# i3drobotics/i3dr_stereo_camera-ros

Measured on AMD Instinct MI355X. Metric: stereo pairs/sec + ms/frame, 1920×1080 D=256 8-path SGM, 1/2/4/8 MI355X, higher is better.
Workload: dtype u8

## Files before the change

### i3dr_stereo_camera-ros_amd/csrc/census_sgm.hip

```cpp
#include "sgm_device.h"

#include <atomic>
#include <string>

#ifndef SGM_WPE
#define SGM_WPE 4
#endif
#ifndef SGM_WPE32
#define SGM_WPE32 4
#endif
#ifndef SGM_NT_STORE
#define SGM_NT_STORE 1
#endif
#ifndef SGM_NT_LOAD
#define SGM_NT_LOAD 1
#endif
#ifndef SGM_EXP
#define SGM_EXP 0
#endif
#if SGM_EXP != 0 && !defined(SGM_EXPERIMENT_BUILD)
#error "SGM_EXP builds give invalid results: define SGM_EXPERIMENT_BUILD as well (never in a release build)"
#endif
#ifndef SGM_LRPRIO_HW
#define SGM_LRPRIO_HW 37
// ... 124 lines not shown
    } else if constexpr (DPL == 4) {
        const uint32_t v = __builtin_amdgcn_perm(L[1], L[0], 0x06040200u);
        if constexpr (SGM_NT_STORE) __builtin_nontemporal_store(v, (uint32_t*)dst);
        else *(uint32_t*)dst = v;
    } else if constexpr (DPL == 8) {
        typedef unsigned int v2u __attribute__((ext_vector_type(2)));
        const v2u v = {__builtin_amdgcn_perm(L[1], L[0], 0x06040200u), __builtin_amdgcn_perm(L[3], L[2], 0x06040200u)};
        if constexpr (SGM_NT_STORE) __builtin_nontemporal_store(v, (v2u*)dst);
        else *(v2u*)dst = v;
    } else {
        typedef unsigned int v4u __attribute__((ext_vector_type(4)));
#pragma unroll
        for (int q = 0; q < DPL / 16; q++) {
            const v4u v = {__builtin_amdgcn_perm(L[8 * q + 1], L[8 * q + 0], 0x06040200u),
                           __builtin_amdgcn_perm(L[8 * q + 3], L[8 * q + 2], 0x06040200u),
                           __builtin_amdgcn_perm(L[8 * q + 5], L[8 * q + 4], 0x06040200u),
                           __builtin_amdgcn_perm(L[8 * q + 7], L[8 * q + 6], 0x06040200u)};
            v4u* d = (v4u*)(q == 0 ? dst : dst_hi);
            if constexpr (SGM_NT_STORE) __builtin_nontemporal_store(v, d);
            else *d = v;
        }
    }
}

constexpr uint32_t kBaseP = 0x6400u, kBaseP2 = 0x64006400u;
constexpr uint32_t kInfP = 0x7000u, kInfP2 = 0x70007000u;

__device__ __forceinline__ uint32_t pk_min3_p(uint32_t a, uint32_t b, uint32_t c)
{
    typedef _Float16 h2_t __attribute__((ext_vector_type(2)));
    const h2_t r = __builtin_elementwise_minimum(
        __builtin_elementwise_minimum(__builtin_bit_cast(h2_t, a), __builtin_bit_cast(h2_t, b)), __builtin_bit_cast(h2_t, c));
    return __builtin_bit_cast(uint32_t, r);
}
__device__ __forceinline__ uint32_t pk_max(uint32_t a, uint32_t b) { return as_u(__builtin_elementwise_max(as_v2(a), as_v2(b))); }

__device__ __forceinline__ uint32_t bcnt_acc(uint32_t x, uint32_t acc)
{
    uint32_t r;
    asm("v_bcnt_u32_b32 %0, %1, %2" : "=v"(r) : "v"(x), "v"(acc));
    return r;
}
__device__ __forceinline__ uint32_t ham_acc(uint64_t a, uint64_t b, uint32_t acc)
{
    const uint64_t x = a ^ b;
    return bcnt_acc((uint32_t)(x >> 32), bcnt_acc((uint32_t)x, acc));
}

__device__ __forceinline__ uint32_t pk_shl(uint32_t a, int sh)
{
    return as_u(as_v2(a) << (u16x2_t){(unsigned short)sh, (unsigned short)sh});
}
__device__ __forceinline__ uint32_t pk_subs(uint32_t a, uint32_t b) { return as_u(__builtin_elementwise_sub_sat(as_v2(a), as_v2(b))); }
template <int DPL, int LPL = 16>
__device__ __forceinline__ void p16_relative(const uint32_t (&Labs)[DPL / 2], uint32_t (&Lr)[DPL / 2])
{
    constexpr int M = DPL / 2;
    uint32_t mn = Labs[0];
#pragma unroll
    for (int i = 1; i < M; i += 2) mn = (i + 1 < M) ? pk_min3_p(mn, Labs[i], Labs[i + 1]) : pk_min(mn, Labs[i]);
    mn = line_min_u32<LPL>(pk_min(mn, alignbit16(mn, mn)));
    uint32_t off = mn - kBaseP2;
    asm("" : "+v"(off));
#pragma unroll
    for (int i = 0; i < M; i++) Lr[i] = Labs[i] - off;
}

template <int DPL, bool EXACT, int LPL = 16, typename F>
__device__ __forceinline__ void p16_step(uint32_t (&Lr)[DPL / 2], uint64_t cl, F crk, uint32_t P1P1, uint32_t P2P2,
                                         const uint32_t (&imask)[DPL / 2], uint32_t (&Labs)[DPL / 2])
{
    constexpr int M = DPL / 2;
    constexpr int SH = LPL == 8 ? 2 : 1;
    uint32_t q[M];
#pragma unroll
    for (int i = 0; i < M; i++) q[i] = Lr[i] + P1P1;
    const uint32_t X = LPL == 32 ? line32_shr1(q[M - 1], kInfP2) : row_shr_n<SH>(q[M - 1], kInfP2);
    const uint32_t Y = LPL == 32 ? line32_shl1(q[0], kInfP2) : row_shl_n<SH>(q[0], kInfP2);
    uint32_t Oprev = alignbit16(q[0], X);
#pragma unroll
    for (int i = 0; i < M; i++) {
        const uint32_t Onext = (i + 1 < M) ? alignbit16(q[i + 1], q[i]) : alignbit16(Y, q[M - 1]);
        const uint32_t t = pk_min(pk_min3_p(Oprev, Onext, Lr[i]), P2P2);
        const uint32_t c1 = ham_acc(cl, crk(2 * i + 1), 0u);
        uint32_t L = ham_acc(cl, crk(2 * i), t) + (c1 << 16);
        if (!EXACT) L = pk_max(L, imask[i]);
        Labs[i] = L;
        Oprev = Onext;
    }
    p16_relative<DPL, LPL>(Labs, Lr);
}

template <int DPL, bool EXACT>
__device__ __forceinline__ void make_imask(int p, int D, uint32_t (&imask)[DPL / 2], uint32_t (&start)[DPL / 2])
{
#pragma unroll
    for (int i = 0; i < DPL / 2; i++) {
        const int d = p * DPL + 2 * i;
        imask[i] = EXACT ? 0u : ((d < D ? 0u : kInfP) | (d + 1 < D ? 0u : kInfP << 16));
        start[i] = imask[i] | kBaseP2;
    }
}

struct PathLaunch16 {
    int xb_lo[6];
    const uint8_t* bnd[2];
    size_t bnd_slot;
};
__host__ __device__ constexpr int bnd_slot_of(int dir) { return dir <= 1 ? 0 : (dir == 2 || dir == 4 ? 1 : 2); }
__host__ __device__ constexpr uint32_t path_item(int dir, int lb, int f = 0)
{
    return ((uint32_t)dir << 24) | ((uint32_t)f << 22) | (uint32_t)lb;
}

template <typename T>
__device__ __forceinline__ T pick4(const T (&a)[kMaxGroup], int f)
{
    return f == 0 ? a[0] : f == 1 ? a[1] : f == 2 ? a[2] : a[3];
}

constexpr int kWG = 256;

template <int DPL16>
struct LineCfg {
    static constexpr int LPL = (DPL16 == 32 && SGM_P32) ? 32 : 16;
    static constexpr int DPL = DPL16 * 16 / LPL;
    static constexpr int HROWS = 4 * (64 / LPL);
};

struct HChunk16 {
    uint64_t cl, inj;
};

template <int DPL, int DX, int LPL>
__device__ __forceinline__ HChunk16 hload16(const uint64_t* cLr, const uint64_t* cRr, const Geom& g, int chunk,
                                            int i16)
{
    const int i = chunk * 16 + i16;
    const int x = DX > 0 ? g.minX1 + i : g.maxX1 - 1 - i;
    HChunk16 c;
    c.cl = cLr[min(max(x, 0), g.W - 1)];
    const int xr = DX > 0 ? x + 1 - g.minD : x - g.minD - LPL * DPL;
    c.inj = cRr[min(max(xr, 0), g.W - 1)];
    return c;
}

template <int DPL, bool EXACT, int DX, bool PRIO = false, int LPL = 16>
__device__ __forceinline__ void p16_horiz(const uint64_t* __restrict__ cL, const uint64_t* __restrict__ cR,
                                          uint8_t* __restrict__ V, uint8_t* __restrict__ trash, const Geom& g,
                                          int y0)
{
    static_assert(LPL == 16 || LPL == 32, "horizontal scans: 16- or 32-lane lines");
    constexpr int M = DPL / 2;
    constexpr int U = DPL > 16 ? DPL : 16;
    const int lane = threadIdx.x & 63;
    const int r = lane / LPL, p = lane % LPL;
    const int y = y0 + r;
    const bool rowok = y < g.H;
    const int yc = min(y, g.H - 1);
    const uint64_t* cLr = cL + (size_t)yc * g.W;
    const uint64_t* cRr = cR + (size_t)yc * g.W;
    uint32_t imask[M], start[M];
    make_imask<DPL, EXACT>(p, g.D, imask, start);
    const uint32_t P1P1 = (uint32_t)g.P1 * 0x10001u, P2P2 = ((uint32_t)g.P2 + kBaseP) * 0x10001u;
    const int n = g.width1;
    const int xfirst = DX > 0 ? g.minX1 : g.maxX1 - 1;
    uint64_t cr[DPL];
#pragma unroll
    for (int k = 0; k < DPL; k++) cr[k] = cRr[min(max(xfirst - g.minD - p * DPL - k, 0), g.W - 1)];
    uint32_t Lr[M];
#pragma unroll
    for (int i = 0; i < M; i++) Lr[i] = start[i];
    uint8_t* rowbase = V + (size_t)yc * g.width1 * g.D + p * DPL;
    uint8_t* tr = trash + lane * DPL;
    const bool lane_ok = rowok && (EXACT || p * DPL < g.D);
    const bool hi_ok = EXACT || p * DPL + 16 < g.D;
    HChunk16 cur = hload16<DPL, DX, LPL>(cLr, cRr, g, 0, lane & 15);
    HChunk16 nxt = cur;
    for (int b = 0; b * U < n; b++) {
        if constexpr (PRIO) lr_prio(((n - b * U) * SGM_LRPRIO_HW) >> 6, g.H);
        static_for<0, U>([&](auto tc) {
            constexpr int t = decltype(tc)::value;
            if constexpr (t % 16 == 0) nxt = hload16<DPL, DX, LPL>(cLr, cRr, g, (b * U + t) / 16 + 1, lane & 15);
            const int i = b * U + t;
            const uint64_t cl = row_bcast_u64<t % 16>(cur.cl);
            const uint64_t inj = row_bcast_u64<t % 16>(cur.inj);
            uint32_t Labs[M];
            p16_step<DPL, EXACT, LPL>(Lr, cl, [&](int k) { return cr[DX > 0 ? ((k - t) % DPL + DPL) % DPL : (k + t) % DPL]; },
                                      P1P1, P2P2, imask, Labs);
            const int x1 = DX > 0 ? i : n - 1 - i;
            const bool ok = lane_ok && i < n;
            uint8_t* dst = ok ? rowbase + (size_t)x1 * g.D : tr;
            store_pairs<DPL>(dst, (ok && hi_ok) ? dst + 16 : tr + 16, Labs);
            if constexpr (DX > 0) {
                constexpr int ph = ((DPL - 1 - t) % DPL + DPL) % DPL;
                cr[ph] = LPL == 32 ? line32_shr1_u64(cr[ph], inj) : row_shr1_u64(cr[ph], inj);
            } else {
                constexpr int ph = t % DPL;
                cr[ph] = LPL == 32 ? line32_shl1_u64(cr[ph], inj) : row_shl1_u64(cr[ph], inj);
            }
            if constexpr (t % 16 == 15) cur = nxt;
        });
    }
}

template <int DPL, int LPL>
struct RowSeg {
    static constexpr int NL = kWG / LPL;
    static constexpr int NSEG = LPL * DPL + NL - 1;
    static constexpr int NPAD = LPL >= 16 ? NSEG + NSEG / 16 + 1 : NSEG + 4 * (NSEG / 32) + 4;
    static constexpr int NTOT = NSEG + NL;
    static constexpr int NLOAD = (NTOT + kWG - 1) / kWG;
    static constexpr int BUF = NPAD + NL + kWG;
    static __device__ __forceinline__ int phys(int e) { return LPL >= 16 ? e + (e >> 4) : e + 4 * (e >> 5); }
};
template <int DPL16>
// ... 53 lines not shown
    }
}

template <int DPL, bool EXACT, int LPL>
__device__ __forceinline__ void p16_seed(const uint8_t* src, const uint32_t (&imask)[DPL / 2], uint32_t (&Lr)[DPL / 2])
{
    uint32_t wd[(DPL + 3) / 4], Labs[DPL / 2];
    wload<DPL>(src, wd);
#pragma unroll
    for (int i = 0; i < DPL / 2; i++) {
        const uint32_t pr = __builtin_amdgcn_perm(0u, wd[i / 2], (i & 1) ? 0x0c030c02u : 0x0c010c00u);
        Labs[i] = pr | kBaseP2;
        if (!EXACT) Labs[i] = pk_max(Labs[i], imask[i]);
    }
    p16_relative<DPL, LPL>(Labs, Lr);
}

struct UpWta {
    const uint8_t* vols;
    size_t vol_bytes;
    uint64_t* res;
};
struct WtaPix { int best, minS, d16; bool rej; };
template <int DPL, bool EXACT>
__device__ __forceinline__ WtaPix wta_pix16(const uint32_t (&E)[(DPL + 3) / 4], const uint32_t (&O)[(DPL + 3) / 4],
                                            int p, const Geom& g, float inv_u, uint32_t* srow);
template <int DPL, bool EXACT>
__device__ __forceinline__ void wta_emask(int p, const Geom& g, uint32_t (&emaskE)[(DPL + 3) / 4],
                                          uint32_t (&emaskO)[(DPL + 3) / 4]);
template <int DPL>
__host__ __device__ constexpr size_t upwta_lds_bytes() { return (size_t)8 * 2 * RowSeg<DPL, 16>::BUF + (size_t)16 * 32 * ((DPL + 3) / 4) * 4; }

template <int DPL, bool EXACT, int LPL, bool FUSE = false, bool PRIO = false>
__device__ __forceinline__ void p16_rows(const uint64_t* __restrict__ cL, const uint64_t* __restrict__ cR,
                                         uint8_t* __restrict__ V, uint8_t* __restrict__ trash, const Geom& g, int dir,
                                         int xb, const PathLaunch16& pl, uint64_t* lds, const UpWta& uw = UpWta{})
{
    static_assert(!FUSE || LPL == 16, "up+WTA blocks use 16 lanes per line (the WTA layout)");
    using RS = RowSeg<DPL, LPL>;
    constexpr int M = DPL / 2;
    constexpr int NL = RS::NL;
    const int tid = threadIdx.x;
    const int lane = tid & 63, w = tid >> 6;
    const int r = lane >> 4;
    const int p = LPL == 32 ? lane & 31 : LPL == 16 ? lane & 15 : (lane & 15) >> 1;
    const int j = LPL == 32 ? 2 * w + (lane >> 5) : LPL == 16 ? 4 * w + r : 8 * w + 2 * r + (lane & 1);
    const int rx = dir_rx(dir), ry = dir_ry(dir);
    int s0, s1;
    if (rx == 0) { s0 = 0; s1 = g.H; }
    else if (rx > 0) { s0 = max(0, g.minX1 - xb - (NL - 1)); s1 = min(g.H, g.maxX1 - xb); }
    else { s0 = max(0, xb - g.maxX1 + 1); s1 = min(g.H, xb + NL - g.minX1); }
    if (s0 >= s1) return;
    uint32_t imask[M], start[M];
    make_imask<DPL, EXACT>(p, g.D, imask, start);
    const uint32_t P1P1 = (uint32_t)g.P1 * 0x10001u, P2P2 = ((uint32_t)g.P2 + kBaseP) * 0x10001u;
    uint32_t Lr[M];
#pragma unroll
    for (int i = 0; i < M; i++) Lr[i] = start[i];
    bool pv = false;
    const uint8_t* bnd = pl.bnd[ry > 0 ? 0 : 1];
    if (bnd && s0 == 0) {
        const int x = xb + j, xp = x - rx;
        const bool cont = x >= g.minX1 && x < g.maxX1 && xp >= g.minX1 && xp < g.maxX1;
        const int xs = min(max(xp, g.minX1), g.maxX1 - 1) - g.minX1;
        uint32_t Ls[M];
        p16_seed<DPL, EXACT, LPL>(bnd + bnd_slot_of(dir) * pl.bnd_slot + (size_t)xs * g.D + p * DPL, imask, Ls);
#pragma unroll
        for (int i = 0; i < M; i++) Lr[i] = cont ? Ls[i] : Lr[i];
        pv = cont;
    }
    const bool lane_act = EXACT || p * DPL < g.D;
    const bool hi_ok = EXACT || p * DPL + 16 < g.D;
    uint8_t* const tr = trash + (tid & 63) * DPL;
    const int e_hi = j + (LPL - p) * DPL - 1;

    uint64_t* buf0 = lds;
    uint64_t* buf1 = lds + RS::BUF;
    uint64_t R0[RS::NLOAD], R1[RS::NLOAD], R2[RS::NLOAD], R3[RS::NLOAD];
    const SegAddr<DPL, LPL> sa = seg_addr<DPL, LPL>(cL, cR, g, tid);
    seg_load<DPL, LPL>(R0, sa, g, rx, ry, xb, s0);
    seg_store<DPL, LPL>(buf0, R0, tid);
    seg_load<DPL, LPL>(R1, sa, g, rx, ry, xb, min(s0 + 1, s1 - 1));
    seg_load<DPL, LPL>(R2, sa, g, rx, ry, xb, min(s0 + 2, s1 - 1));
    seg_load<DPL, LPL>(R3, sa, g, rx, ry, xb, min(s0 + 3, s1 - 1));
    __syncthreads();

    constexpr int NWD = (DPL + 3) / 4;
    uint32_t vw[7][NWD], emaskE[NWD], emaskO[NWD];
    uint32_t* srow = (uint32_t*)(lds + 2 * RS::BUF) + j * 32 * NWD;
    const float inv_u = 1.0f / (float)max(100 - g.uniq, 1);
    const uint32_t voff = (uint32_t)((min(max(xb + j, g.minX1), g.maxX1 - 1) - g.minX1) * g.D + (lane_act ? p * DPL : 0));
    auto vload = [&](int s) {
        const uint8_t* rb = uw.vols + (size_t)max(g.H - 1 - s, 0) * g.width1 * g.D;
#pragma unroll
        for (int k = 0; k < 7; k++) wload_buf<DPL>(rb + (size_t)(k == 0 ? 0 : k + 1) * uw.vol_bytes, voff, vw[k]);
    };
    if constexpr (FUSE) {
        wta_emask<DPL, EXACT>(p, g, emaskE, emaskO);
        vload(s0);
    }
    auto step = [&](int s, const uint64_t* bufc) {
        const int x = xb + j + rx * s;
        const bool valid = s < s1 && x >= g.minX1 && x < g.maxX1;
        const int y = ry > 0 ? s : g.H - 1 - s;
        const uint64_t cl = bufc[RS::NPAD + j];
        uint32_t Labs[M];
        uint32_t E[NWD], O[NWD];
        if constexpr (FUSE) {
#pragma unroll
            for (int jj = 0; jj < NWD; jj++) {
                uint32_t e = 0, o = 0;
#pragma unroll
                for (int k = 0; k < 7; k++) {
                    e += vw[k][jj] & 0x00FF00FFu;
                    o += __builtin_amdgcn_perm(0u, vw[k][jj], 0x0c030c01u);
                }
                asm("" : "+v"(e), "+v"(o));
                E[jj] = e;
                O[jj] = o;
            }
        }
        const uint32_t P2x = pv ? P2P2 : kBaseP2;
        if constexpr (FUSE) __builtin_amdgcn_sched_barrier(0);
        p16_step<DPL, EXACT, LPL>(Lr, cl, [&](int k) { return bufc[RS::phys(e_hi - k)]; }, P1P1, P2x, imask, Labs);
        if constexpr (FUSE) {
            __builtin_amdgcn_sched_barrier(0);
#pragma unroll
            for (int jj = 0; jj < NWD; jj++) {
                const uint32_t a = Labs[2 * jj], b = 2 * jj + 1 < M ? Labs[2 * jj + 1] : 0u;
                E[jj] = (E[jj] + __builtin_amdgcn_perm(b, a, 0x0c040c00u)) | emaskE[jj];
                O[jj] = (O[jj] + __builtin_amdgcn_perm(b, a, 0x0c060c02u)) | emaskO[jj];
            }
            vload(s + 1);
            __builtin_amdgcn_sched_barrier(0);
            const WtaPix px = wta_pix16<DPL, EXACT>(E, O, p, g, inv_u, srow);
            const uint64_t v = (uint64_t)(uint16_t)(px.rej ? g.invalid : px.d16) |
                               ((uint64_t)(uint16_t)(px.rej ? -1 : px.best) << 16) | ((uint64_t)(uint16_t)px.minS << 32);
            const __amdgpu_buffer_rsrc_t rr =
                __builtin_amdgcn_make_buffer_rsrc((void*)(uw.res + (size_t)y * g.W), 0, g.W * 8, 0x00020000);
            typedef unsigned int v2u __attribute__((ext_vector_type(2)));
            __builtin_amdgcn_raw_buffer_store_b64(__builtin_bit_cast(v2u, v), rr,
                                                  (valid && p == 0) ? (uint32_t)x * 8u : 0x80000000u, 0, 2);
        } else {
            const bool ok = valid && lane_act && !((SGM_EXP & 2) && dir == 1);
            uint8_t* const vrow = V + (size_t)min(max(y, 0), g.H - 1) * g.width1 * g.D;
            uint8_t* const dst = ok ? vrow + (uint32_t)((x - g.minX1) * g.D + p * DPL) : tr;
            store_pairs<DPL>(dst, (ok && hi_ok) ? dst + 16 : tr + 16, Labs);
        }
        pv = valid;
    };
    auto body = [&](int s, const uint64_t* bcur, uint64_t* bnext, uint64_t (&Rnext)[RS::NLOAD],
                    uint64_t (&Rfree)[RS::NLOAD]) {
        seg_load<DPL, LPL>(Rfree, sa, g, rx, ry, xb, min(s + 4, s1 - 1));
        step(s, bcur);
        seg_store<DPL, LPL>(bnext, Rnext, tid);
        __syncthreads();
    };
    for (int s = s0; s < s1; s += 4) {
        if constexpr (PRIO) lr_prio(rx != 0 ? ((s1 - s) * SGM_LRPRIO_DIAG) >> 6 : s1 - s, g.H);
        body(s, buf0, buf1, R1, R0);
        body(s + 1, buf1, buf0, R2, R1);
        body(s + 2, buf0, buf1, R3, R2);
        body(s + 3, buf1, buf0, R0, R3);
    }
}

template <int DPL>
__host__ __device__ constexpr int rows_lds_codes() { return 2 * RowSeg<RowsCfg<DPL>::DPL, RowsCfg<DPL>::LPL>::BUF; }

template <int DPL, bool EXACT, bool PRIO = false>
__device__ __forceinline__ void paths_block16(const PathFrames& pf, size_t vol_bytes, size_t trash_off,
                                              const Geom& g, const PathLaunch16& pl, uint32_t it, uint64_t* lds)
{
    using RC = RowsCfg<DPL>;
    using HC = LineCfg<DPL>;
    const int dir = (int)(it >> 24);
    const int f = (int)((it >> 22) & 3u);
    const int lb = (int)(it & 0x3FFFFFu);
    if (f >= pf.n || ((pf.skip_dirs >> dir) & 1u)) return;
    const uint64_t* cL = pick4(pf.cL, f);
    const uint64_t* cR = pick4(pf.cR, f);
    uint8_t* V = pick4(pf.vols, f) + (size_t)dir * vol_bytes;
    uint8_t* trash = V + trash_off;
    const int y0 = lb * HC::HROWS + (64 / HC::LPL) * (threadIdx.x >> 6);
    if (dir == 6) p16_horiz<HC::DPL, EXACT, 1, PRIO, HC::LPL>(cL, cR, V, trash, g, y0);
    else if (dir == 7) p16_horiz<HC::DPL, EXACT, -1, PRIO, HC::LPL>(cL, cR, V, trash, g, y0);
    else p16_rows<RC::DPL, EXACT, RC::LPL, false, PRIO>(cL, cR, V, trash, g, dir, pl.xb_lo[dir] + lb * RC::NL, pl, lds);
}

__device__ __forceinline__ void trace_record(uint64_t* trace, uint64_t tag, uint64_t t0)
{
    const uint64_t t1 = __builtin_amdgcn_s_memrealtime();
    const uint32_t hw = __builtin_amdgcn_s_getreg((4 << 0) | (0 << 6) | (31 << 11));
    const uint32_t xcc = __builtin_amdgcn_s_getreg((20 << 0) | (0 << 6) | (15 << 11));
    uint64_t* r = trace + ((size_t)blockIdx.x * 4 + (threadIdx.x >> 6)) * 4;
    r[0] = tag | ((uint64_t)blockIdx.x << 32); r[1] = ((uint64_t)xcc << 32) | hw; r[2] = t0; r[3] = t1;
}

template <int DPL, bool EXACT>
__global__ __launch_bounds__(kWG) __attribute__((amdgpu_waves_per_eu(DPL >= 32 && !SGM_P32 ? SGM_WPE32 : SGM_WPE)))
void k_census_paths16(PathFrames pf, size_t vol_bytes, size_t trash_off, Geom g, PathLaunch16 pl,
                      const uint32_t* __restrict__ items, uint64_t* __restrict__ trace)
{
    __shared__ uint64_t lds[rows_lds_codes<DPL>()];
    const uint64_t t0 = trace ? __builtin_amdgcn_s_memrealtime() : 0;
    paths_block16<DPL, EXACT, true>(pf, vol_bytes, trash_off, g, pl, items[blockIdx.x], lds);
    if (trace && (threadIdx.x & 63) == 0)
        trace_record(trace, items[blockIdx.x], t0);
}

template <int DPL>
__host__ __device__ constexpr size_t wta_key_bytes(int W)
{
    return (size_t)kWG * 8 * ((DPL + 3) / 4) > (size_t)4 * W ? (size_t)kWG * 8 * ((DPL + 3) / 4) : (size_t)4 * W;
}
template <int DPL>
__host__ __device__ constexpr size_t wta_lds_bytes(int W) { return wta_key_bytes<DPL>(W) + RowLds::rest_bytes(W); }

template <int DPL, bool EXACT>
__device__ __forceinline__ WtaPix wta_pix16(const uint32_t (&E)[(DPL + 3) / 4], const uint32_t (&O)[(DPL + 3) / 4],
                                            int p, const Geom& g, float inv_u, uint32_t* srow)
{
    constexpr int NWD = (DPL + 3) / 4;
    constexpr int KB = DPL > 16 ? 5 : 4;
    constexpr uint32_t KMASK = (1u << KB) - 1;
    uint32_t km = 0xFFFFFFFFu;
#pragma unroll
    for (int j = 0; j < NWD; j++) {
        const uint32_t ke = pk_shl(E[j], KB) | (((uint32_t)(4 * j + 2) << 16) | (uint32_t)(4 * j));
        const uint32_t ko = pk_shl(O[j], KB) | (((uint32_t)(4 * j + 3) << 16) | (uint32_t)(4 * j + 1));
        km = pk_min(km, pk_min(ke, ko));
    }
    km = pk_min(km, alignbit16(km, km)) & 0xFFFFu;
    const uint32_t kmin = row_min_u32(((km >> KB) << 9) | (uint32_t)(p * DPL + (int)(km & KMASK)));
    WtaPix r;
    const int best = (int)(kmin & 511u);
    const int minS = (int)(kmin >> 9);
#pragma unroll
    for (int j = 0; j < NWD; j++) { srow[p * 2 * NWD + j] = E[j]; srow[p * 2 * NWD + NWD + j] = O[j]; }
    auto s_at = [&](int d) {
        const int kk = d % DPL;
        const uint32_t v = srow[(d / DPL) * 2 * NWD + (kk & 1) * NWD + (kk >> 2)];
        return (int)((v >> (16 * ((kk >> 1) & 1))) & 0xFFFFu);
    };
    const int sm = s_at(max(best - 1, 0)), sp = s_at(min(best + 1, 16 * DPL - 1));
    int T = 0;
    if (g.uniq < 100) {
        if (minS > 0) {
            const int num = minS * 100 - 1, den = 100 - g.uniq;
            int q = (int)((float)num * inv_u);
            q += (q + 1) * den <= num ? 1 : 0;
            q -= q * den > num ? 1 : 0;
            T = min(q + 1, 8 * 255 + 1);
        }
    } else {
        T = (minS == 0 && g.uniq > 100) ? 1 : 0;
    }
    const uint32_t TT = (uint32_t)T * 0x10001u;
    uint32_t acc = 0;
#pragma unroll
    for (int j = 0; j < NWD; j++) acc += pk_subs(TT, E[j]) + pk_subs(TT, O[j]);
    const int tot = (int)row_sum_u32(__builtin_amdgcn_sad_u16(acc, 0u, 0u));
    const int win = max(T - minS, 0) + (best > 0 ? max(T - sm, 0) : 0) + (best < g.D - 1 ? max(T - sp, 0) : 0);
    int outside = tot - win;
    if (g.uniq >= 100) {
        const int nwin = 1 + (best > 0 ? 1 : 0) + (best < g.D - 1 ? 1 : 0);
        outside = minS > 0 ? g.D - nwin : (g.uniq > 100 ? (g.D - nwin) - outside : 0);
    }
    r.rej = outside > 0;
    const int den = max(sm + sp - 2 * minS, 1);
    const bool use = g.subpix && best > 0 && best < g.D - 1;
    r.d16 = best * 16 + (use ? tdiv_rcp((sm - sp) * 16 + den, 2 * den) : 0) + g.minD * 16;
    r.best = best;
    r.minS = minS;
    return r;
}

template <int DPL, bool EXACT>
__device__ __forceinline__ void wta_emask(int p, const Geom& g, uint32_t (&emaskE)[(DPL + 3) / 4],
                                          uint32_t (&emaskO)[(DPL + 3) / 4])
{
#pragma unroll
    for (int j = 0; j < (DPL + 3) / 4; j++) {
        auto bad = [&](int k) { return k >= DPL || (!EXACT && p * DPL + k >= g.D); };
        emaskE[j] = (bad(4 * j) ? 0xFFFFu : 0u) | (bad(4 * j + 2) ? 0xFFFF0000u : 0u);
        emaskO[j] = (bad(4 * j + 1) ? 0xFFFFu : 0u) | (bad(4 * j + 3) ? 0xFFFF0000u : 0u);
    }
}

template <int DPL, bool EXACT, typename OutT = int16_t>
__device__ __forceinline__ void wta_row16(const uint8_t* __restrict__ vols, size_t vol_bytes, const Geom& g,
                                          OutT* __restrict__ out, size_t out_stride, int y, uint32_t* lds)
{
    constexpr int NWD = (DPL + 3) / 4;
    uint32_t* sl = lds;
    RowLds R(lds, (char*)lds + wta_key_bytes<DPL>(g.W), g.W);
    const int tid = threadIdx.x, lane = tid & 63;
    const int w = __builtin_amdgcn_readfirstlane(tid >> 6);
    const int r = lane >> 4, p = lane & 15;
    R.init(g, tid, kWG, false);
    const bool lane_act = EXACT || p * DPL < g.D;
    const size_t row0 = (size_t)y * g.width1 * g.D;
    const uint32_t off0 = (uint32_t)(lane_act ? p * DPL : 0);
    uint32_t* srow = sl + (w * 4 + r) * 32 * NWD;
    uint32_t emaskE[NWD], emaskO[NWD];
    wta_emask<DPL, EXACT>(p, g, emaskE, emaskO);
    const float inv_u = 1.0f / (float)max(100 - g.uniq, 1);
    const int n = g.width1;
    const int nq = (n + 3) / 4;
    const uint32_t loff = off0 + (uint32_t)(r * g.D);
    auto load = [&](int q, uint32_t (&v)[8][NWD]) {
        const uint8_t* rowq = vols + row0 + (size_t)(4 * q) * g.D;
#pragma unroll
        for (int vv = 0; vv < 8; vv++) {
            if ((SGM_EXP & 4) && vv == 1) { for (int j = 0; j < NWD; j++) v[vv][j] = 0; continue; }
            wload_buf<DPL>(rowq + (size_t)vv * vol_bytes, loff, v[vv]);
        }
    };
    uint32_t E[NWD], O[NWD];
    auto sum8 = [&](const uint32_t (&v)[8][NWD]) {
#pragma unroll
        for (int j = 0; j < NWD; j++) {
            uint32_t e = 0, o = 0;
#pragma unroll
            for (int vv = 0; vv < 8; vv++) {
                e += v[vv][j] & 0x00FF00FFu;
                o += __builtin_amdgcn_perm(0u, v[vv][j], 0x0c030c01u);
            }
            E[j] = e | emaskE[j];
            O[j] = o | emaskO[j];
        }
    };
    uint32_t nxt[8][NWD];
    load(min(w, nq - 1), nxt);
    sum8(nxt);
    for (int q = w; q < nq; q += 4) {
        load(min(q + 4, nq - 1), nxt);
// ... 55 lines not shown
            tile[i] = v;
            if (rect && ty >= 3 && ty < 3 + kCensusRows && tx >= 4 && tx < 68 && y0 + ty - 3 < H && x0 + tx - 4 < W)
                rect[(size_t)yy * cf.rect_stride + xx] = v;
        }
    } else {
        for (int i = threadIdx.x; i < TH * 72; i += kWG) {
            const int ty = i / 72, tx = i - ty * 72;
            const int yy = min(max(y0 + ty - 3, 0), H - 1), xx = min(max(x0 + tx - 4, 0), W - 1);
            tile[i] = src[(size_t)yy * cf.stride + xx];
        }
    }
    __syncthreads();
    const int tx = threadIdx.x & 63, x = x0 + tx;
    if (x >= W) return;
    for (int ty = threadIdx.x >> 6; ty < kCensusRows; ty += kWG / 64) {
        const int y = y0 + ty;
        if (y >= H) break;
        out[(size_t)y * W + x] = census_code_lds<72>(tile, ty, tx);
    }
}

__global__ __launch_bounds__(kWG) void k_census_tiles(CensusFrames cf, int W, int H)
{
    __shared__ __attribute__((aligned(16))) uint8_t tile[(kCensusRows + 6) * 72];
    census_block(cf, W, H, blockIdx.x, tile);
}

template <int DPL, bool EXACT>
__global__ __launch_bounds__(kWG) __attribute__((amdgpu_waves_per_eu(DPL >= 32 ? SGM_WPE32 : SGM_WPE)))
void k_census_fused16(PathFrames pf, WtaFrames wf, CensusFrames cf, size_t vol_bytes, size_t trash_off, Geom g,
                      PathLaunch16 pl, const uint32_t* __restrict__ items, int n_items, size_t out_stride,
                      int period16, int wta_rows, uint64_t* __restrict__ trace)
{
    extern __shared__ uint64_t lds_dyn64[];
    const uint64_t t0 = trace ? __builtin_amdgcn_s_memrealtime() : 0;
    const int b = blockIdx.x;
    const int n_wta = wta_rows ? g.H * wf.n : 0;
    auto wcount = [&](int bb) {
        int w = period16 > 0 ? min((bb + 1) * 16 / period16, n_wta) : 0;
        return max(w, bb + 1 - n_items);
    };
    int kind = 2, idx = b - n_items - n_wta;
    if (b < n_items + n_wta) {
        const int w = wcount(b);
        const bool is_wta = w > (b > 0 ? wcount(b - 1) : 0);
        kind = is_wta ? 1 : 0;
        idx = is_wta ? w - 1 : b - w;
    }
    if (kind == 0) {
        const uint32_t it = items[idx];
        if constexpr (DPL > 16) {
            paths_block16<DPL, EXACT>(pf, vol_bytes, trash_off, g, pl, it, lds_dyn64);
        } else if ((it >> 24) == 8u) {
            using RC = RowsCfg<DPL>;
            const int f = (int)((it >> 22) & 3u);
            if (f < wf.n) {
#if SGM_UPWTA_PRIO
                __builtin_amdgcn_s_setprio(SGM_UPWTA_PRIO);
#endif
                const UpWta uw{pick4(wf.vols, f), vol_bytes, pick4(wf.res, f)};
                p16_rows<DPL, EXACT, 16, true>(pick4(wf.cL, f), pick4(wf.cR, f), nullptr, nullptr, g, 1,
                                               pl.xb_lo[1] + (int)(it & 0x3FFFFFu) * 16, pl, lds_dyn64, uw);
            }
        } else {
            paths_block16<DPL, EXACT>(pf, vol_bytes, trash_off, g, pl, it, lds_dyn64);
        }
    } else if (kind == 1) {
        wta_block16<DPL, EXACT>(wf, vol_bytes, g, out_stride, idx, (uint32_t*)lds_dyn64);
    } else {
        census_block(cf, g.W, g.H, idx, (uint8_t*)lds_dyn64);
    }
    if (trace && (threadIdx.x & 63) == 0)
        trace_record(trace, (kind == 0 ? items[idx] : 0u) | ((uint64_t)kind << 62), t0);
}

__global__ __launch_bounds__(kWG) void k_census_rowfin(WtaFrames wf, Geom g, size_t out_stride)
{
    extern __shared__ uint32_t lds_dyn[];
    const int f = blockIdx.x / g.H, y = blockIdx.x - f * g.H;
    const uint64_t* res = pick4(wf.res, f) + (size_t)y * g.W;
    RowLds R(lds_dyn, g.W);
    R.init(g, threadIdx.x, kWG, true);
    for (int x = g.minX1 + threadIdx.x; x < g.maxX1; x += kWG) {
        const uint64_t v = __builtin_nontemporal_load(res + x);
        R.drow[x] = (int16_t)(uint16_t)v;
        R.bst[x] = (int16_t)(uint16_t)(v >> 16);
        R.mins[x] = (uint16_t)(v >> 32);
    }
    row_finish(g, threadIdx.x, kWG, R.drow, R.bst, R.mins, R.key, (int16_t*)R.mins, pick4(wf.out, f) + (size_t)y * out_stride);
}

hipError_t launch_census(const uint8_t* L, const uint8_t* R, size_t stride, int W, int H, uint64_t* cL,
                         uint64_t* cR, hipStream_t st)
{
    dim3 grid((W + 63) / 64, (H + 3) / 4, R ? 2 : 1);
    hipLaunchKernelGGL(k_census9x7, grid, dim3(256), 0, st, L, R, stride, W, H, cL, cR);
    return hipGetLastError();
}

static int dpl16_for(int D) { return D <= 32 ? 2 : D <= 64 ? 4 : D <= 128 ? 8 : D <= 256 ? 16 : 32; }
static int rows_lines(int D)
{
    switch (dpl16_for(D)) {
    case 2: return RowsCfg<2>::NL;
    case 4: return RowsCfg<4>::NL;
    case 8: return RowsCfg<8>::NL;
    case 16: return RowsCfg<16>::NL;
    default: return RowsCfg<32>::NL;
    }
}
static int hscan_rows(int D) { return dpl16_for(D) == 32 ? LineCfg<32>::HROWS : LineCfg<16>::HROWS; }

PathLaunch16 make_path_launch16(const Geom& g)
{
    PathLaunch16 pl{};
    for (int dir = 0; dir < 6; dir++) pl.xb_lo[dir] = g.minX1 - (dir_rx(dir) > 0 ? g.H - 1 : 0);
    return pl;
}

int census_path_items(const Geom& g, unsigned dir_mask, int n_slots, int group, uint32_t* out, int cap, int up_group)
{
    struct Item { int len; uint32_t code; };
    std::vector<Item> v;
    const PathLaunch16 pl = make_path_launch16(g);
    group = std::min(std::max(group, 1), kMaxGroup);
    up_group = std::min(std::max(up_group, 0), kMaxGroup);
    {
        const int NL = 16;
        const int nb = (g.maxX1 - pl.xb_lo[1] + NL - 1) / NL;
        for (int b = 0; b < nb; b++)
            for (int f = 0; f < up_group; f++) v.push_back({4 * g.H + 4 * g.W, path_item(8, b, f)});
    }
    for (int dir = 0; dir < 8; dir++) {
        if (!((dir_mask >> dir) & 1u)) continue;
        if (dir >= 6) {
            const int nb = (g.H + hscan_rows(g.D) - 1) / hscan_rows(g.D);
            for (int b = 0; b < nb; b++)
                for (int f = 0; f < group; f++) v.push_back({g.width1, path_item(dir, b, f)});
            continue;
        }
        const int rx = dir_rx(dir);
        const int hi = g.maxX1 + (rx < 0 ? g.H - 1 : 0);
        const int NL = rows_lines(g.D);
        const int nb = (hi - pl.xb_lo[dir] + NL - 1) / NL;
        for (int b = 0; b < nb; b++) {
            const int xb = pl.xb_lo[dir] + b * NL;
            int s0, s1;
            if (rx == 0) { s0 = 0; s1 = g.H; }
            else if (rx > 0) { s0 = std::max(0, g.minX1 - xb - (NL - 1)); s1 = std::min(g.H, g.maxX1 - xb); }
            else { s0 = std::max(0, xb - g.maxX1 + 1); s1 = std::min(g.H, xb + NL - g.minX1); }
            for (int f = 0; f < group; f++) v.push_back({std::max(s1 - s0, 0), path_item(dir, b, f)});
        }
    }
// ... 161 lines not shown
```

### i3dr_stereo_camera-ros_amd/csrc/sgm_api.cpp

```cpp
#include <hip/hip_runtime.h>

#include <algorithm>
#include <chrono>
#include <condition_variable>
#include <cstdio>
#include <cstdlib>
#include <cstring>
#include <functional>
#include <mutex>
#include <string>
#include <thread>
#include <vector>

#include "sgm_device.h"
#include "sgm_hip.h"

namespace sgm {
hipError_t launch_census(const uint8_t*, const uint8_t*, size_t, int, int, uint64_t*, uint64_t*, hipStream_t);
int census_path_items(const Geom&, unsigned, int, int, uint32_t*, int, int up_group = 0);
hipError_t launch_census_paths(const PathFrames&, size_t, const Geom&, const uint32_t*, int, hipStream_t,
                               const uint8_t* = nullptr, const uint8_t* = nullptr, size_t = 0);
hipError_t launch_census_wta(const WtaFrames&, size_t, const Geom&, size_t, hipStream_t);
hipError_t launch_rectify_map(const double*, const double*, const double*, int, int, float*, float*, size_t,
                              hipStream_t);
hipError_t launch_remap_cubic(const uint8_t*, size_t, int, int, const float*, const float*, size_t, int, int,
                              const int16_t*, uint8_t*, size_t, hipStream_t);
void cubic_table(int16_t*);
bool rectify_inverse(const double*, const double*, double*);
hipError_t launch_census_tiles(const CensusFrames&, int, int, hipStream_t);
hipError_t launch_census_fused(const PathFrames&, const WtaFrames&, const CensusFrames&, size_t, const Geom&,
                               const uint32_t*, int, size_t, bool, hipStream_t);
hipError_t launch_census_rowfin(const WtaFrames&, const Geom&, size_t, hipStream_t);
hipError_t launch_median3(const int16_t*, size_t, int16_t*, size_t, int, int, hipStream_t);
hipError_t launch_speckle(const int16_t*, size_t, int16_t*, size_t, int, int, int, int, int, int*, int*, hipStream_t);
hipError_t launch_fill16(int16_t*, size_t, int, int, int, hipStream_t);
hipError_t launch_to_f32(const int16_t*, size_t, float*, size_t, int, int, hipStream_t);
hipError_t launch_disp_to_msg(const int16_t*, size_t, int, int, float, float, float*, size_t, hipStream_t);
hipError_t launch_depth_points(const float*, size_t, int, int, const float*, double, double, const uint8_t*, size_t,
                               int, float*, size_t, float4*, int, int*, int*, hipStream_t);
hipError_t launch_ocv_cost(const uint8_t*, const uint8_t*, size_t, const Geom&, int, uint8_t*, int16_t*, int16_t*,
                           hipStream_t);
bool ocv_cost_takes_fused(const Geom&);
hipError_t launch_ocv_paths(const int16_t*, const int16_t*, void*, size_t, const Geom&, int, hipStream_t,
                            int skipdir = -1);
hipError_t launch_ocv_vwta(const int16_t*, const int16_t*, const void*, size_t, int, const Geom&, uint64_t*, hipStream_t);
int ocv_vwta_dir(int ndir);
hipError_t launch_ocv_wta(const int16_t*, const void*, size_t, int, const Geom&, int16_t*, size_t, hipStream_t);
int ocv_evol_mode(const Geom&, int, int);
}

using sgm::Geom;

#ifndef SGM_VOL_PAD_BYTES
#define SGM_VOL_PAD_BYTES 0
#endif
#ifndef SGM_IO_PRIO
#define SGM_IO_PRIO 1
#endif

namespace {

constexpr size_t kAlign = 256;
constexpr size_t kTrashBytes = 4096;
inline size_t align_up(size_t v) { return (v + kAlign - 1) / kAlign * kAlign; }

int make_geom(const sgm_params& p, int W, int H, Geom& g, std::string& err)
{
    if (W <= 0 || H <= 0) { err = "image size must be positive"; return SGM_ERR_ARG; }
    if (W > 32767 || H > 32767) { err = "image larger than 32767 pixels"; return SGM_ERR_UNSUPPORTED; }
    if (p.mode < SGM_MODE_OCV_SGBM5 || p.mode > SGM_MODE_CENSUS8) { err = "unknown mode"; return SGM_ERR_PARAM; }
    if (p.num_disparities <= 0 || p.num_disparities % 16 != 0) {
        err = "numDisparities must be a positive multiple of 16 (OpenCV: CV_Assert(D % 16 == 0))";
// ... 1882 lines not shown
int sgm_stage_launches(const sgm_handle* h, int i)
{
    if (!h || i < 0 || i >= h->nstages) return 0;
    int c = 0;
    for (const auto& r : h->launches) c += (r.stage == i && r.ev1 != r.ev0) ? 1 : 0;
    return c;
}

int sgm_debug_census(sgm_handle* h, const uint8_t* img, int W, int H, size_t stride, uint64_t* out)
{
    if (!h || !img || !out || W <= 0 || H <= 0 || stride < (size_t)W) return SGM_ERR_ARG;
    std::lock_guard<std::mutex> lk(h->mu);
    int rc = ensure_stream(h);
    if (rc || (rc = order_after_last(h, h->stream))) return rc;
    const size_t WH = (size_t)W * H;
    if ((rc = ensure_ws(h, align_up(WH) + WH * 8))) return rc;
    char* ws = (char*)h->ws.base;
    HIP_TRY(hipMemcpy2DAsync(ws, W, img, stride, W, H, hipMemcpyHostToDevice, h->stream), "H2D");
    HIP_TRY(sgm::launch_census((const uint8_t*)ws, nullptr, W, W, H, (uint64_t*)(ws + align_up(WH)), nullptr,
                               h->stream), "census");
    HIP_TRY(hipMemcpyAsync(out, ws + align_up(WH), WH * 8, hipMemcpyDeviceToHost, h->stream), "D2H");
    HIP_TRY(hipStreamSynchronize(h->stream), "sync");
    return SGM_OK;
}

int sgm_debug_census_path(sgm_handle* h, const uint8_t* L, const uint8_t* R, int W, int H, size_t stride, int dir,
                          uint8_t* vol)
{
    if (!h || !L || !R || !vol || dir < 0 || dir > 7) return SGM_ERR_ARG;
    std::lock_guard<std::mutex> lk(h->mu);
    if (h->params.mode != SGM_MODE_CENSUS8) return fail(h, SGM_ERR_PARAM, "census mode required");
    Geom g;
    Layout l;
    int rc = prepare(h, W, H, true, g, l);
    if (rc || (rc = order_after_last(h, h->stream))) return rc;
    if (g.width1 <= 0) return SGM_OK;
    char* ws = (char*)h->ws.base;
    HIP_TRY(hipMemcpy2DAsync(ws + l.inL, W, L, stride, W, H, hipMemcpyHostToDevice, h->stream), "H2D");
    HIP_TRY(hipMemcpy2DAsync(ws + l.inR, W, R, stride, W, H, hipMemcpyHostToDevice, h->stream), "H2D");
    uint64_t* cL = (uint64_t*)(ws + l.cL[0]);
    uint64_t* cR = (uint64_t*)(ws + l.cR[0]);
    uint8_t* vols = (uint8_t*)(ws + l.vols[0]);
    HIP_TRY(sgm::launch_census((const uint8_t*)(ws + l.inL), (const uint8_t*)(ws + l.inR), W, W, H, cL, cR, h->stream),
            "census");
    const uint32_t* items;
    const int n_items = path_items(h, l, g, 1u << dir, 1, h->stream, &items);
    if (n_items < 0) return n_items;
    sgm::PathFrames pf{};
    pf.cL[0] = cL; pf.cR[0] = cR; pf.vols[0] = vols; pf.n = 1;
    HIP_TRY(sgm::launch_census_paths(pf, l.vol_bytes, g, items, n_items, h->stream), "paths");
    const size_t cells = (size_t)g.width1 * g.H * g.D;
    HIP_TRY(hipMemcpyAsync(vol, vols + (size_t)dir * l.vol_bytes, cells, hipMemcpyDeviceToHost, h->stream), "D2H");
    HIP_TRY(hipStreamSynchronize(h->stream), "sync");
    return SGM_OK;
}

int sgm_debug_ocv_cost(sgm_handle* h, const uint8_t* L, const uint8_t* R, int W, int H, size_t stride, int16_t* cost)
{
    if (!h || !L || !R || !cost) return SGM_ERR_ARG;
    std::lock_guard<std::mutex> lk(h->mu);
    if (h->params.mode == SGM_MODE_CENSUS8) return fail(h, SGM_ERR_PARAM, "OCV mode required");
    Geom g;
    Layout l;
    int rc = prepare(h, W, H, true, g, l);
    if (rc || (rc = order_after_last(h, h->stream))) return rc;
    if (g.width1 <= 0) return SGM_OK;
    char* ws = (char*)h->ws.base;
    HIP_TRY(hipMemcpy2DAsync(ws + l.inL, W, L, stride, W, H, hipMemcpyHostToDevice, h->stream), "H2D");
    HIP_TRY(hipMemcpy2DAsync(ws + l.inR, W, R, stride, W, H, hipMemcpyHostToDevice, h->stream), "H2D");
    int16_t* A = (int16_t*)(ws + l.bufA);
    int16_t* B = (int16_t*)(ws + l.bufB);
    int flag = 0;
    if (g.wide == 2) {
        g.ovf = (int*)(ws + l.ovf);
        HIP_TRY(hipMemsetAsync(g.ovf, 0, sizeof(int), h->stream), "hipMemsetAsync");
    }
    HIP_TRY(sgm::launch_ocv_cost((const uint8_t*)(ws + l.inL), (const uint8_t*)(ws + l.inR), W, g,
                                 h->params.mode == SGM_MODE_OCV_HH8, (uint8_t*)(ws + l.planes), A, B, h->stream),
            "ocv_cost");
    if (g.wide == 2) HIP_TRY(hipMemcpyAsync(&flag, g.ovf, sizeof(int), hipMemcpyDeviceToHost, h->stream), "D2H flag");
    HIP_TRY(hipStreamSynchronize(h->stream), "sync");
    (void)flag;
    const size_t cells = (size_t)g.width1 * g.H * g.D;
    HIP_TRY(hipMemcpyAsync(cost, A, cells * 2, hipMemcpyDeviceToHost, h->stream), "D2H");
    HIP_TRY(hipStreamSynchronize(h->stream), "sync");
    return SGM_OK;
}

static int debug_post(sgm_handle* h, int16_t* disp, int W, int H, int which, int nv, int ms, int md)
{
    if (!h || !disp || W <= 0 || H <= 0) return SGM_ERR_ARG;
    std::lock_guard<std::mutex> lk(h->mu);
    int rc = ensure_stream(h);
    if (rc || (rc = order_after_last(h, h->stream))) return rc;
    const size_t WH = (size_t)W * H;
    if ((rc = ensure_ws(h, align_up(WH * 2) * 2 + align_up(WH * 4) * 2))) return rc;
    char* ws = (char*)h->ws.base;
    int16_t* a = (int16_t*)ws;
    int16_t* b = (int16_t*)(ws + align_up(WH * 2));
    int* lab = (int*)(ws + 2 * align_up(WH * 2));
    int* cnt = (int*)(ws + 2 * align_up(WH * 2) + align_up(WH * 4));
    HIP_TRY(hipMemcpyAsync(a, disp, WH * 2, hipMemcpyHostToDevice, h->stream), "H2D");
    if (which == 0) {
        HIP_TRY(sgm::launch_median3(a, W, b, W, W, H, h->stream), "median3");
        HIP_TRY(hipMemcpyAsync(disp, b, WH * 2, hipMemcpyDeviceToHost, h->stream), "D2H");
    } else {
// ... 31 lines not shown
```

### i3dr_stereo_camera-ros_amd/csrc/sgm_device.h

```cpp
#pragma once
#include <hip/hip_runtime.h>
#include <stdint.h>

#include "sgm_hip.h"

#include <type_traits>

namespace sgm {

template <int B, int E, typename F>
__host__ __device__ __forceinline__ void static_for(F&& f) {
    if constexpr (B < E) {
        f(std::integral_constant<int, B>{});
        static_for<B + 1, E>(f);
    }
}

constexpr int kCodeMargin = 1024;
constexpr int kInf = 0x3FFF;

struct Geom {
    int W, H;
    int minD, D;
    int minX1, maxX1;
    int width1;
    int P1, P2;
    int uniq;
    int disp12;
    int subpix, lr;
    int invalid;
    int SW2, SH2, ftzero;
    int wide;
    int* ovf;
    int compat;
    int ovf_thr;
    int evol;
};

__host__ __device__ inline size_t ocv_planes_bytes(int W, int H) { return ((size_t)W * H * 4 + 255) / 256 * 256; }
__host__ __device__ inline size_t ocv_planes_total(int W, int H) { return ocv_planes_bytes(W, H) + (size_t)W * H * 16; }

__host__ __device__ inline size_t ocv_vol_elems(size_t cells, size_t es) { return (cells * es + 255) / 256 * 256 / es; }
#ifndef SGM_LRPRIO_SCALE
#define SGM_LRPRIO_SCALE 8
#endif
__device__ __forceinline__ void lr_prio(int rem, int span)
{
    const int lvl = min(3, SGM_LRPRIO_SCALE * rem / (span + 1));
    if (lvl >= 3) __builtin_amdgcn_s_setprio(3);
    else if (lvl == 2) __builtin_amdgcn_s_setprio(2);
    else if (lvl == 1) __builtin_amdgcn_s_setprio(1);
    else __builtin_amdgcn_s_setprio(0);
}

template <bool FLAGGED>
__device__ __forceinline__ bool ocv_gate_skip(const Geom& g)
{
    return g.wide == 2 && ((*g.ovf != 0) != FLAGGED);
}
__device__ __forceinline__ bool ocv_flagged(const Geom& g)
{
    return g.wide == 1 || (g.wide == 2 && *g.ovf != 0);
}

__host__ __device__ constexpr int dir_rx(int i) { return i == 2 || i == 4 || i == 6 ? 1 : (i == 3 || i == 5 || i == 7 ? -1 : 0); }
__host__ __device__ constexpr int dir_ry(int i) { return i == 0 || i == 2 || i == 3 ? 1 : (i == 1 || i == 4 || i == 5 ? -1 : 0); }

__device__ __forceinline__ int dpp_shr1(int v, int old) {
    return __builtin_amdgcn_update_dpp(old, v, 0x138, 0xf, 0xf, false);
}
__device__ __forceinline__ int dpp_shl1(int v, int old) {
    return __builtin_amdgcn_update_dpp(old, v, 0x130, 0xf, 0xf, false);
}
__device__ __forceinline__ uint64_t dpp_shr1_u64(uint64_t v, uint64_t old) {
    int lo = dpp_shr1((int)(uint32_t)v, (int)(uint32_t)old);
    int hi = dpp_shr1((int)(uint32_t)(v >> 32), (int)(uint32_t)(old >> 32));
    return ((uint64_t)(uint32_t)hi << 32) | (uint32_t)lo;
}
__device__ __forceinline__ uint64_t dpp_shl1_u64(uint64_t v, uint64_t old) {
    int lo = dpp_shl1((int)(uint32_t)v, (int)(uint32_t)old);
    int hi = dpp_shl1((int)(uint32_t)(v >> 32), (int)(uint32_t)(old >> 32));
    return ((uint64_t)(uint32_t)hi << 32) | (uint32_t)lo;
}

__device__ __forceinline__ int wave_min(int v) {
    v = min(v, __builtin_amdgcn_update_dpp(v, v, 0xB1, 0xf, 0xf, false));
    v = min(v, __builtin_amdgcn_update_dpp(v, v, 0x4E, 0xf, 0xf, false));
    v = min(v, __builtin_amdgcn_update_dpp(v, v, 0x124, 0xf, 0xf, false));
    v = min(v, __builtin_amdgcn_update_dpp(v, v, 0x128, 0xf, 0xf, false));
    int a = __builtin_amdgcn_readlane(v, 0), b = __builtin_amdgcn_readlane(v, 16);
    int c = __builtin_amdgcn_readlane(v, 32), d = __builtin_amdgcn_readlane(v, 48);
    return min(min(a, b), min(c, d));
}

__device__ __forceinline__ int popc64(uint64_t a) { return __builtin_popcountll(a); }

__device__ __forceinline__ int tdiv(int num, int den) {
    int q = (int)__builtin_truncf((float)num / (float)den);
    int r = num - q * den;
    if (num >= 0) { if (r >= den) q++; else if (r < 0) q--; }
    else          { if (r <= -den) q--; else if (r > 0) q++; }
    return q;
}

template <int DPL>
__device__ __forceinline__ int pick(const int (&S)[DPL], int k) {
    int r = S[0];
#pragma unroll
    for (int i = 1; i < DPL; i++) r = (k == i) ? S[i] : r;
    return r;
}

__device__ __forceinline__ uint64_t readlane64(uint64_t v, int lane) {
    const uint32_t lo = (uint32_t)__builtin_amdgcn_readlane((int)(uint32_t)v, lane);
    const uint32_t hi = (uint32_t)__builtin_amdgcn_readlane((int)(uint32_t)(v >> 32), lane);
    return ((uint64_t)hi << 32) | lo;
}
// ... 294 lines not shown
```

Baseline: 727.9.

## Reorder disparity pairs in packed registers to avoid alignbit shuffles in path step

Changes the packing of disparities in the 16-bit pair registers so each register holds d and d+G/2 within a group instead of adjacent d, d+1. Neighbour disparities then sit in adjacent registers, and the P1 min in the path recurrence needs alignbit16 only at group edges. The volume byte order, the imask/emask, the WTA index decode and the debug volume readback (un-permuted on the host) are updated to match. It also hoists the result row pointer and scalarises the volume base pointer in the fused up+WTA path. The cost is more complex indexing in the WTA code and a host-side permutation in the debug path.

```diff
diff --git a/i3dr_stereo_camera-ros_amd/csrc/census_sgm.hip b/i3dr_stereo_camera-ros_amd/csrc/census_sgm.hip
--- a/i3dr_stereo_camera-ros_amd/csrc/census_sgm.hip
+++ b/i3dr_stereo_camera-ros_amd/csrc/census_sgm.hip
@@ -200,6 +200,8 @@
     return as_u(as_v2(a) << (u16x2_t){(unsigned short)sh, (unsigned short)sh});
 }
 __device__ __forceinline__ uint32_t pk_subs(uint32_t a, uint32_t b) { return as_u(__builtin_elementwise_sub_sat(as_v2(a), as_v2(b))); }
+__host__ __device__ constexpr int line_group(int dpl, int lpl) { return pair_group(lpl == 8 ? dpl / 2 : dpl); }
+
 template <int DPL, int LPL = 16>
 __device__ __forceinline__ void p16_relative(const uint32_t (&Labs)[DPL / 2], uint32_t (&Lr)[DPL / 2])
 {
@@ -220,32 +222,34 @@
 {
     constexpr int M = DPL / 2;
     constexpr int SH = LPL == 8 ? 2 : 1;
+    constexpr int G = line_group(DPL, LPL), G2 = G / 2;
     uint32_t q[M];
 #pragma unroll
     for (int i = 0; i < M; i++) q[i] = Lr[i] + P1P1;
     const uint32_t X = LPL == 32 ? line32_shr1(q[M - 1], kInfP2) : row_shr_n<SH>(q[M - 1], kInfP2);
     const uint32_t Y = LPL == 32 ? line32_shl1(q[0], kInfP2) : row_shl_n<SH>(q[0], kInfP2);
-    uint32_t Oprev = alignbit16(q[0], X);
 #pragma unroll
     for (int i = 0; i < M; i++) {
-        const uint32_t Onext = (i + 1 < M) ? alignbit16(q[i + 1], q[i]) : alignbit16(Y, q[M - 1]);
+        const int i0 = i / G2 * G2, il = i - i0;
+        const uint32_t Oprev = il > 0 ? q[i - 1] : alignbit16(q[i0 + G2 - 1], i0 > 0 ? q[i0 - 1] : X);
+        const uint32_t Onext = il + 1 < G2 ? q[i + 1] : alignbit16(i0 + G2 < M ? q[i0 + G2] : Y, q[i0]);
         const uint32_t t = pk_min(pk_min3_p(Oprev, Onext, Lr[i]), P2P2);
-        const uint32_t c1 = ham_acc(cl, crk(2 * i + 1), 0u);
-        uint32_t L = ham_acc(cl, crk(2 * i), t) + (c1 << 16);
+        const uint32_t c1 = ham_acc(cl, crk(pair_d(G, i, 1)), 0u);
+        uint32_t L = ham_acc(cl, crk(pair_d(G, i, 0)), t) + (c1 << 16);
         if (!EXACT) L = pk_max(L, imask[i]);
         Labs[i] = L;
-        Oprev = Onext;
     }
     p16_relative<DPL, LPL>(Labs, Lr);
 }
 
-template <int DPL, bool EXACT>
+template <int DPL, bool EXACT, int LPL = 16>
 __device__ __forceinline__ void make_imask(int p, int D, uint32_t (&imask)[DPL / 2], uint32_t (&start)[DPL / 2])
 {
+    constexpr int G = line_group(DPL, LPL);
 #pragma unroll
     for (int i = 0; i < DPL / 2; i++) {
-        const int d = p * DPL + 2 * i;
-        imask[i] = EXACT ? 0u : ((d < D ? 0u : kInfP) | (d + 1 < D ? 0u : kInfP << 16));
+        const int dlo = p * DPL + pair_d(G, i, 0), dhi = p * DPL + pair_d(G, i, 1);
+        imask[i] = EXACT ? 0u : ((dlo < D ? 0u : kInfP) | (dhi < D ? 0u : kInfP << 16));
         start[i] = imask[i] | kBaseP2;
     }
 }
@@ -309,7 +313,7 @@
     const uint64_t* cLr = cL + (size_t)yc * g.W;
     const uint64_t* cRr = cR + (size_t)yc * g.W;
     uint32_t imask[M], start[M];
-    make_imask<DPL, EXACT>(p, g.D, imask, start);
+    make_imask<DPL, EXACT, LPL>(p, g.D, imask, start);
     const uint32_t P1P1 = (uint32_t)g.P1 * 0x10001u, P2P2 = ((uint32_t)g.P2 + kBaseP) * 0x10001u;
     const int n = g.width1;
     const int xfirst = DX > 0 ? g.minX1 : g.maxX1 - 1;
@@ -469,7 +473,7 @@
     else { s0 = max(0, xb - g.maxX1 + 1); s1 = min(g.H, xb + NL - g.minX1); }
     if (s0 >= s1) return;
     uint32_t imask[M], start[M];
-    make_imask<DPL, EXACT>(p, g.D, imask, start);
+    make_imask<DPL, EXACT, LPL>(p, g.D, imask, start);
     const uint32_t P1P1 = (uint32_t)g.P1 * 0x10001u, P2P2 = ((uint32_t)g.P2 + kBaseP) * 0x10001u;
     uint32_t Lr[M];
 #pragma unroll
@@ -507,8 +511,10 @@
     uint32_t* srow = (uint32_t*)(lds + 2 * RS::BUF) + j * 32 * NWD;
     const float inv_u = 1.0f / (float)max(100 - g.uniq, 1);
     const uint32_t voff = (uint32_t)((min(max(xb + j, g.minX1), g.maxX1 - 1) - g.minX1) * g.D + (lane_act ? p * DPL : 0));
+    uint64_t vols0 = (uint64_t)uw.vols;
+    if constexpr (FUSE) asm volatile("" : "+s"(vols0));
     auto vload = [&](int s) {
-        const uint8_t* rb = uw.vols + (size_t)max(g.H - 1 - s, 0) * g.width1 * g.D;
+        const uint8_t* rb = (const uint8_t*)vols0 + (size_t)max(g.H - 1 - s, 0) * g.width1 * g.D;
 #pragma unroll
         for (int k = 0; k < 7; k++) wload_buf<DPL>(rb + (size_t)(k == 0 ? 0 : k + 1) * uw.vol_bytes, voff, vw[k]);
     };
@@ -516,6 +522,7 @@
         wta_emask<DPL, EXACT>(p, g, emaskE, emaskO);
         vload(s0);
     }
+    const uint64_t* resrow = FUSE ? uw.res + (size_t)(g.H - 1 - s0) * g.W : nullptr;
     auto step = [&](int s, const uint64_t* bufc) {
         const int x = xb + j + rx * s;
         const bool valid = s < s1 && x >= g.minX1 && x < g.maxX1;
@@ -553,8 +560,8 @@
             const WtaPix px = wta_pix16<DPL, EXACT>(E, O, p, g, inv_u, srow);
             const uint64_t v = (uint64_t)(uint16_t)(px.rej ? g.invalid : px.d16) |
                                ((uint64_t)(uint16_t)(px.rej ? -1 : px.best) << 16) | ((uint64_t)(uint16_t)px.minS << 32);
-            const __amdgpu_buffer_rsrc_t rr =
-                __builtin_amdgcn_make_buffer_rsrc((void*)(uw.res + (size_t)y * g.W), 0, g.W * 8, 0x00020000);
+            const __amdgpu_buffer_rsrc_t rr = __builtin_amdgcn_make_buffer_rsrc((void*)resrow, 0, g.W * 8, 0x00020000);
+            resrow -= g.W;
             typedef unsigned int v2u __attribute__((ext_vector_type(2)));
             __builtin_amdgcn_raw_buffer_store_b64(__builtin_bit_cast(v2u, v), rr,
                                                   (valid && p == 0) ? (uint32_t)x * 8u : 0x80000000u, 0, 2);
@@ -641,11 +648,18 @@
     constexpr int NWD = (DPL + 3) / 4;
     constexpr int KB = DPL > 16 ? 5 : 4;
     constexpr uint32_t KMASK = (1u << KB) - 1;
+    constexpr int G = pair_group(DPL);
+    auto kof = [](int b) { return (uint32_t)(b < DPL ? vol_byte_d(G, b) : b) & KMASK; };
     uint32_t km = 0xFFFFFFFFu;
 #pragma unroll
     for (int j = 0; j < NWD; j++) {
-        const uint32_t ke = pk_shl(E[j], KB) | (((uint32_t)(4 * j + 2) << 16) | (uint32_t)(4 * j));
-        const uint32_t ko = pk_shl(O[j], KB) | (((uint32_t)(4 * j + 3) << 16) | (uint32_t)(4 * j + 1));
+        uint32_t ce = (kof(4 * j + 2) << 16) | kof(4 * j), co = (kof(4 * j + 3) << 16) | kof(4 * j + 1);
+        uint32_t ke, ko;
+        if constexpr (EXACT && DPL >= 4) {
+            asm("" : "+s"(ce), "+s"(co));
+            ke = (E[j] << KB) | ce; ko = (O[j] << KB) | co;
+        }
+        else { ke = pk_shl(E[j], KB) | ce; ko = pk_shl(O[j], KB) | co; }
         km = pk_min(km, pk_min(ke, ko));
     }
     km = pk_min(km, alignbit16(km, km)) & 0xFFFFu;
@@ -656,7 +670,7 @@
 #pragma unroll
     for (int j = 0; j < NWD; j++) { srow[p * 2 * NWD + j] = E[j]; srow[p * 2 * NWD + NWD + j] = O[j]; }
     auto s_at = [&](int d) {
-        const int kk = d % DPL;
+        const int kk = vol_d_byte(G, d % DPL);
         const uint32_t v = srow[(d / DPL) * 2 * NWD + (kk & 1) * NWD + (kk >> 2)];
         return (int)((v >> (16 * ((kk >> 1) & 1))) & 0xFFFFu);
     };
@@ -699,7 +713,7 @@
 {
 #pragma unroll
     for (int j = 0; j < (DPL + 3) / 4; j++) {
-        auto bad = [&](int k) { return k >= DPL || (!EXACT && p * DPL + k >= g.D); };
+        auto bad = [&](int b) { return b >= DPL || (!EXACT && p * DPL + vol_byte_d(pair_group(DPL), b) >= g.D); };
         emaskE[j] = (bad(4 * j) ? 0xFFFFu : 0u) | (bad(4 * j + 2) ? 0xFFFF0000u : 0u);
         emaskO[j] = (bad(4 * j + 1) ? 0xFFFFu : 0u) | (bad(4 * j + 3) ? 0xFFFF0000u : 0u);
     }
@@ -861,7 +875,6 @@
         if constexpr (DPL > 16) {
             paths_block16<DPL, EXACT>(pf, vol_bytes, trash_off, g, pl, it, lds_dyn64);
         } else if ((it >> 24) == 8u) {
-            using RC = RowsCfg<DPL>;
             const int f = (int)((it >> 22) & 3u);
             if (f < wf.n) {
 #if SGM_UPWTA_PRIO
@@ -908,6 +921,7 @@
 }
 
 static int dpl16_for(int D) { return D <= 32 ? 2 : D <= 64 ? 4 : D <= 128 ? 8 : D <= 256 ? 16 : 32; }
+int census_vol_group(int D) { return pair_group(dpl16_for(D)); }
 static int rows_lines(int D)
 {
     switch (dpl16_for(D)) {
diff --git a/i3dr_stereo_camera-ros_amd/csrc/sgm_api.cpp b/i3dr_stereo_camera-ros_amd/csrc/sgm_api.cpp
--- a/i3dr_stereo_camera-ros_amd/csrc/sgm_api.cpp
+++ b/i3dr_stereo_camera-ros_amd/csrc/sgm_api.cpp
@@ -18,6 +18,7 @@
 namespace sgm {
 hipError_t launch_census(const uint8_t*, const uint8_t*, size_t, int, int, uint64_t*, uint64_t*, hipStream_t);
 int census_path_items(const Geom&, unsigned, int, int, uint32_t*, int, int up_group = 0);
+int census_vol_group(int D);
 hipError_t launch_census_paths(const PathFrames&, size_t, const Geom&, const uint32_t*, int, hipStream_t,
                                const uint8_t* = nullptr, const uint8_t* = nullptr, size_t = 0);
 hipError_t launch_census_wta(const WtaFrames&, size_t, const Geom&, size_t, hipStream_t);
@@ -2006,6 +2007,12 @@
     const size_t cells = (size_t)g.width1 * g.H * g.D;
     HIP_TRY(hipMemcpyAsync(vol, vols + (size_t)dir * l.vol_bytes, cells, hipMemcpyDeviceToHost, h->stream), "D2H");
     HIP_TRY(hipStreamSynchronize(h->stream), "sync");
+    const int G = sgm::census_vol_group(g.D);
+    uint8_t t[16];
+    for (size_t c = 0; c + G <= cells; c += G) {
+        for (int b = 0; b < G; b++) t[sgm::vol_byte_d(G, b)] = vol[c + b];
+        memcpy(vol + c, t, G);
+    }
     return SGM_OK;
 }
 
diff --git a/i3dr_stereo_camera-ros_amd/csrc/sgm_device.h b/i3dr_stereo_camera-ros_amd/csrc/sgm_device.h
--- a/i3dr_stereo_camera-ros_amd/csrc/sgm_device.h
+++ b/i3dr_stereo_camera-ros_amd/csrc/sgm_device.h
@@ -63,6 +63,17 @@
     return g.wide == 1 || (g.wide == 2 && *g.ovf != 0);
 }
 
+__host__ __device__ constexpr int pair_group(int dpl16) { return dpl16 < 16 ? dpl16 : 16; }
+__host__ __device__ constexpr int pair_d(int g, int i, int hi)
+{
+    return i / (g / 2) * g + i % (g / 2) + hi * (g / 2);
+}
+__host__ __device__ constexpr int vol_byte_d(int g, int b) { return pair_d(g, b >> 1, b & 1); }
+__host__ __device__ constexpr int vol_d_byte(int g, int k)
+{
+    return k / g * g + 2 * (k % g % (g / 2)) + k % g / (g / 2);
+}
+
 __host__ __device__ constexpr int dir_rx(int i) { return i == 2 || i == 4 || i == 6 ? 1 : (i == 3 || i == 5 || i == 7 ? -1 : 0); }
 __host__ __device__ constexpr int dir_ry(int i) { return i == 0 || i == 2 || i == 3 ? 1 : (i == 1 || i == 4 || i == 5 ? -1 : 0); }
 
```

New measurement: 748.7 (median of 6 runs). 1.03x the previous value.
